# bluenote-1577/skani

Hardware: AMD Instinct MI355X
Metric: genome-pairs/sec (triangle, ~5 Mbp genomes) (higher is better)
Workload: dtype u64

## Files before the change

skani_amd/csrc/chain_dp.h:

```cpp
#pragma once

template <class Co> struct Blk { Co q, r; uint32_t cr; int32_t score; uint32_t root, depth; };

template <int PB, class W>
__global__ __launch_bounds__(256) void chain_dp_kernel(uint32_t n_slots, const Chunk* chunks, uint32_t band, const typename W::Co* anc_q, const typename W::Co* anc_r, unsigned long long* best,
                                                       uint32_t* st ) {
    using Co = typename W::Co; using Blk = skh::Blk<Co>;
    const uint32_t slot = blockIdx.x * (blockDim.x >> 6) + (threadIdx.x >> 6);
    if (slot >= n_slots) return;
    const Chunk ck = chunks[slot];
    if (ck.a_end <= ck.a_begin) return;
    const int l = (int)lane_id();
    Blk prev[PB > 0 ? PB : 1];
#pragma unroll
    for (int b = 0; b < (PB > 0 ? PB : 1); b++) prev[b] = Blk{0, 0, 0, 0, 0, 0};
    for (uint32_t base = ck.a_begin; base < ck.a_end; base += 64) {
        const uint32_t t = base + (uint32_t)l;
        const bool valid = t < ck.a_end;
        Blk cur;
        Co av_q = 0, av_r = 0;
        if (valid) { av_q = anc_q[t]; av_r = anc_r[t]; }
        cur.q = av_q; cur.r = av_r >> 1; cur.cr = (uint32_t)(av_r & 1u);
        cur.score = 0; cur.root = t; cur.depth = 1;
        uint32_t ptr = t;
        uint32_t jlo = base - ck.a_begin > band ? base - band : ck.a_begin;
        const uint32_t jhi = ck.a_end < base + 64 ? ck.a_end : base + 64;
        {
            const Co q_base = anc_q[base];
            uint32_t lo = jlo, hi = base;
            while (lo < hi) { const uint32_t mid = (lo + hi) >> 1; if (anc_q[mid] + BP_CHAIN_BAND < q_base) lo = mid + 1; else hi = mid; }
            jlo = lo;
        }
        for (uint32_t j = jlo; j < jhi; j++) {
            Co qj, rj; uint32_t crj; int32_t sj;
            if (j >= base) {
                const int ln = (int)(j - base);
                const uint32_t pj = wave_readlane(ptr, ln);
                uint32_t rootj = j, depthj = 1;
                if (pj != j) {
                    if (pj >= base) { rootj = wave_readlane(cur.root, (int)(pj - base)); depthj = wave_readlane(cur.depth, (int)(pj - base)) + 1; }
                    else if (PB == 0) { rootj = __atomic_load_n(&st[3 * (size_t)pj + 1], __ATOMIC_RELAXED); depthj = __atomic_load_n(&st[3 * (size_t)pj + 2], __ATOMIC_RELAXED) + 1; }
                    else {
#pragma unroll
                        for (int b = 0; b < PB; b++) {
                            const uint32_t bb = base - 64u * (uint32_t)(b + 1);
                            if (base >= 64u * (uint32_t)(b + 1) && pj >= bb && pj < bb + 64) { rootj = wave_readlane(prev[b].root, (int)(pj - bb)); depthj = wave_readlane(prev[b].depth, (int)(pj - bb)) + 1; }
                        }
                    }
                }
                if (l == ln) { cur.root = rootj; cur.depth = depthj; }
                qj = wave_readlane(cur.q, ln); rj = wave_readlane(cur.r, ln); crj = wave_readlane(cur.cr, ln); sj = wave_readlane(cur.score, ln);
            } else if (PB == 0) {
                const Co rr = anc_r[j];
                qj = anc_q[j]; rj = rr >> 1; crj = (uint32_t)(rr & 1u); sj = (int32_t)__atomic_load_n(&st[3 * (size_t)j], __ATOMIC_RELAXED);
            } else {
                qj = rj = 0; crj = 0; sj = 0;
#pragma unroll
                for (int b = 0; b < PB; b++) {
                    const uint32_t bb = base - 64u * (uint32_t)(b + 1);
                    if (base >= 64u * (uint32_t)(b + 1) && j >= bb && j < bb + 64) {
                        const int ln = (int)(j - bb);
                        qj = wave_readlane(prev[b].q, ln); rj = wave_readlane(prev[b].r, ln); crj = wave_readlane(prev[b].cr, ln); sj = wave_readlane(prev[b].score, ln);
                    }
                }
            }
            if (valid && t > j && t - j <= band && cur.cr == crj) {
                const Co dq = cur.q - qj;
                const bool rev = (crj & 1u) != 0;
                const bool fwd_ok = rev ? (rj > cur.r) : (cur.r > rj);
                const Co dr = rev ? rj - cur.r : cur.r - rj;
                if (dq != 0 && dq <= BP_CHAIN_BAND && fwd_ok && dr <= (Co)MAX_LIN) {
                    const int32_t gap = (int32_t)dr > (int32_t)dq ? (int32_t)(dr - dq) : (int32_t)(dq - dr);
                    const int32_t s = ANCHOR_SCORE - gap + sj;
                    if (gap <= MAX_GAP && s > 0 && s >= cur.score) { cur.score = s; ptr = j; }
                }
            }
        }
        if (valid) atomicMax(&best[cur.root], best_payload((uint32_t)cur.score, t - ck.a_begin, cur.depth));
        if (PB == 0) {
            if (valid) { __atomic_store_n(&st[3 * (size_t)t], (uint32_t)cur.score, __ATOMIC_RELAXED); __atomic_store_n(&st[3 * (size_t)t + 1], cur.root, __ATOMIC_RELAXED); __atomic_store_n(&st[3 * (size_t)t + 2], cur.depth, __ATOMIC_RELAXED); }
            wave_sync_mem();
        }
#pragma unroll
        for (int b = PB - 1; b > 0; b--) prev[b] = prev[b - 1];
        prev[0] = cur;
    }
}

template <class W> struct EmitCtxT { const typename W::Co *anc_q, *anc_r; const PairDesc* pairs; const WidePair* wide; const uint32_t *pc0, *pi0; uint32_t* ivl_cnt; Interval* ivls; uint32_t* err; };
using EmitCtx = EmitCtxT<Narrow>;
__device__ __forceinline__ bool dp_keep(unsigned long long b) {
    const uint32_t sc = (uint32_t)(b >> 40), na = (uint32_t)(b & 0xFFFFFu);
    return na >= MIN_ANCHORS && (int32_t)sc >= MIN_SCORE;
}
template <class W>
__device__ __forceinline__ void dp_write(const Chunk& ck, uint32_t slot, uint32_t p, uint32_t root, unsigned long long b, const EmitCtxT<W>& ec, uint32_t k) {
    using Co = typename W::Co;
    const uint32_t sc = (uint32_t)(b >> 40), bi = (uint32_t)((b >> 20) & 0xFFFFFu), na = (uint32_t)(b & 0xFFFFFu);
    if (ec.pi0[p] + k >= ec.pi0[p + 1]) { atomicAdd(ec.err, 1u); return; }
    const Co ar_q = ec.anc_q[ck.a_begin + root], ar_r = ec.anc_r[ck.a_begin + root], ab_q = ec.anc_q[ck.a_begin + bi], ab_r = ec.anc_r[ck.a_begin + bi];
    const PairDesc& pd = ec.pairs[p];
    const typename W::Arr bo = W::b_goff(pd, ec.wide, p);
    const Co ra = ar_r >> 1, rb = ab_r >> 1;
    const uint32_t rctg = ctg_of(bo, pd.b_nctg, ra); const Co roff = bo[rctg];
    Co qoff = ck.qoff;
    if constexpr (W::wide) qoff = W::a_goff(pd, ec.wide, p)[ck.qctg];
    Interval iv;
    iv.score = sc; iv.na = na; iv.q0 = (uint32_t)(ar_q - qoff); iv.q1 = (uint32_t)(ab_q - qoff);
    iv.r0 = (uint32_t)((ra < rb ? ra : rb) - roff); iv.r1 = (uint32_t)((ra < rb ? rb : ra) - roff);
    iv.rctg = rctg; iv.qctg = ck.qctg; iv.chunk = slot - ec.pc0[p]; iv.rev = (uint32_t)(ar_r & 1u);
    ec.ivls[ec.pi0[p] + k] = iv;
}
template <class W>
__device__ __forceinline__ void dp_emit(const Chunk& ck, uint32_t slot, uint32_t p, uint32_t root, unsigned long long b, const EmitCtxT<W>& ec) {
    if (dp_keep(b)) dp_write(ck, slot, p, root, b, ec, atomicAdd(&ec.ivl_cnt[p], 1u));
}

constexpr uint32_t DP_ORDER_KEYS = 1024, DP_ORDER_BLOCK = 8192;
__device__ __forceinline__ uint32_t dp_order_key(const Chunk& c) { const uint32_t len = c.a_end - c.a_begin; return (DP_ORDER_KEYS - 1u) - (len >= DP_ORDER_KEYS - 1u ? DP_ORDER_KEYS - 1u : len); }
__global__ __launch_bounds__(256) void dp_order_hist_kernel(uint32_t n_slots, const Chunk* chunks, uint32_t* hist) {
    __shared__ uint32_t lh[DP_ORDER_KEYS];
    for (uint32_t x = threadIdx.x; x < DP_ORDER_KEYS; x += 256) lh[x] = 0;
    __syncthreads();
    const uint32_t e = (blockIdx.x + 1u) * DP_ORDER_BLOCK < n_slots ? (blockIdx.x + 1u) * DP_ORDER_BLOCK : n_slots;
    for (uint32_t i = blockIdx.x * DP_ORDER_BLOCK + threadIdx.x; i < e; i += 256) atomicAdd(&lh[dp_order_key(chunks[i])], 1u);
    __syncthreads();
    for (uint32_t x = threadIdx.x; x < DP_ORDER_KEYS; x += 256) if (lh[x]) atomicAdd(&hist[x], lh[x]);
}
__global__ __launch_bounds__(256) void dp_order_scatter_kernel(uint32_t n_slots, const Chunk* chunks, const uint32_t* hist, uint32_t* cursor, uint32_t* order) {
    __shared__ uint32_t base[DP_ORDER_KEYS], mine[DP_ORDER_KEYS]; __shared__ uint32_t wsum[4];
    const uint32_t t = threadIdx.x;
    uint32_t h[4], s = 0;
#pragma unroll
    for (int x = 0; x < 4; x++) { h[x] = hist[4 * t + x]; s += h[x]; mine[4 * t + x] = 0; }
    const uint32_t incl = wave_incl_scan(s);
    if ((t & 63u) == 63u) wsum[t >> 6] = incl;
    __syncthreads();
    uint32_t off = incl - s;
    for (uint32_t w = 0; w < (t >> 6); w++) off += wsum[w];
#pragma unroll
    for (int x = 0; x < 4; x++) { base[4 * t + x] = off; off += h[x]; }
    __syncthreads();
    constexpr int PER = DP_ORDER_BLOCK / 256;
    const uint32_t i0 = blockIdx.x * DP_ORDER_BLOCK + t;
    uint16_t k[PER], r[PER];
#pragma unroll
    for (int x = 0; x < PER; x++) { const uint32_t i = i0 + 256u * x; k[x] = 0xFFFF; if (i < n_slots) { k[x] = (uint16_t)dp_order_key(chunks[i]); r[x] = (uint16_t)atomicAdd(&mine[k[x]], 1u); } }
    __syncthreads();
#pragma unroll
    for (int x = 0; x < 4; x++) { const uint32_t c = 4 * t + x, n = mine[c]; if (n) base[c] += atomicAdd(&cursor[c], n); }
    __syncthreads();
#pragma unroll
    for (int x = 0; x < PER; x++) if (k[x] != 0xFFFF) order[base[k[x]] + r[x]] = i0 + 256u * x;
}

#ifndef DP_EMIT_Q
#define DP_EMIT_Q 6
#endif
#ifndef DP_LINE
#define DP_LINE 8
#endif
template <int NB, int T, uint32_t DP_LDS_SLOTS, bool EXACT, class W = Narrow>
__global__ __launch_bounds__(T) void chain_dp_thread_kernel(uint32_t n_slots, const Chunk* chunks, const uint32_t* chunk_pair, const uint32_t* order, uint32_t band,
                                                            EmitCtxT<W> ec, unsigned long long* spill_best, uint32_t* spill_rr, uint4* emit_q, uint32_t emit_cap) {
    using Co = typename W::Co;
    __shared__ unsigned long long lds_best[DP_LDS_SLOTS * T];
    __shared__ uint32_t lds_rr[DP_LDS_SLOTS * T];
    const uint32_t C = band + 1, tid = threadIdx.x;
    const uint32_t thr = blockIdx.x * T + tid;
    const uint32_t slot = thr < n_slots ? order[thr] : n_slots;
    const size_t n_thr = (size_t)gridDim.x * T;
    auto get_best = [&](uint32_t c) { return c < DP_LDS_SLOTS ? lds_best[c * T + tid] : spill_best[(size_t)(c - DP_LDS_SLOTS) * n_thr + thr]; };
    auto set_best = [&](uint32_t c, unsigned long long v) { if (c < DP_LDS_SLOTS) lds_best[c * T + tid] = v; else spill_best[(size_t)(c - DP_LDS_SLOTS) * n_thr + thr] = v; };
    auto get_rr = [&](uint32_t c) { return c < DP_LDS_SLOTS ? lds_rr[c * T + tid] : spill_rr[(size_t)(c - DP_LDS_SLOTS) * n_thr + thr]; };
    auto set_rr = [&](uint32_t c, uint32_t v) { if (c < DP_LDS_SLOTS) lds_rr[c * T + tid] = v; else spill_rr[(size_t)(c - DP_LDS_SLOTS) * n_thr + thr] = v; };
    Chunk ck{0, 0, 0, 0, 0, 0};
    if (slot < n_slots) ck = chunks[slot];
    const uint32_t n = ck.a_end - ck.a_begin;
    if (n >= MAX_CHUNK_ANCHORS) { atomicAdd(ec.err, 1u); return; }
    const uint32_t p = n ? chunk_pair[slot] : 0;
    uint32_t nq = 0;
    auto emit = [&](uint32_t root, unsigned long long b) {
        if (!dp_keep(b)) return;
        if (NB <= 40 && nq < emit_cap) { emit_q[(size_t)nq * n_thr + thr] = make_uint4(root, (uint32_t)b, (uint32_t)(b >> 32), 0u); nq++; }
        else dp_emit(ck, slot, p, root, b, ec);
    };
    unsigned long long free_mask = C >= 64 ? ~0ull : ((1ull << C) - 1ull);
    uint32_t rq[NB], rr[NB], rs[NB], rd[NB];
    uint32_t rh[W::wide ? NB : 1];
#pragma unroll
    for (int k = 0; k < NB; k++) { rq[k] = 0; rr[k] = 0; rs[k] = 0; rd[k] = 0; }
#pragma unroll
    for (int k = 0; k < (W::wide ? NB : 1); k++) rh[k] = 0;
    constexpr uint32_t LINE = DP_LINE;
    constexpr int APL = W::wide ? 2 : 4;
    constexpr int LQ = LINE / APL;
    __shared__ uint32_t lds_q[LINE * T], lds_r[LINE * T];
    __shared__ uint32_t lds_rh[W::wide ? LINE * T : 1];
    const uint32_t voff = ck.a_begin & (LINE - 1);
    const uint32_t vtot = n ? n + voff : 0;
    const Co* line_q = ec.anc_q + (ck.a_begin - voff); const Co* line_r = ec.anc_r + (ck.a_begin - voff);
    uint4 pq[LQ], pr[LQ];
#pragma unroll
    for (int j = 0; j < LQ; j++) { pq[j] = make_uint4(0, 0, 0, 0); pr[j] = make_uint4(0, 0, 0, 0); }
    if (vtot) {
#pragma unroll
        for (int j = 0; j < LQ; j++) { pq[j] = *(const uint4*)(line_q + APL * j); pr[j] = *(const uint4*)(line_r + APL * j); }
    }
    for (uint32_t v = 0;; v++) {
        const uint32_t kk = v & (LINE - 1);
        if (kk == 0) {
            if (__ballot(v < vtot) == 0) break;
#pragma unroll
            for (int j = 0; j < LQ; j++) {
                if constexpr (W::wide) {
                    lds_q[(2 * j + 0) * T + tid] = pq[j].x; lds_q[(2 * j + 1) * T + tid] = pq[j].z;
                    lds_r[(2 * j + 0) * T + tid] = pr[j].x; lds_r[(2 * j + 1) * T + tid] = pr[j].z;
                    lds_rh[(2 * j + 0) * T + tid] = pr[j].y; lds_rh[(2 * j + 1) * T + tid] = pr[j].w;
                } else {
                    lds_q[(4 * j + 0) * T + tid] = pq[j].x; lds_q[(4 * j + 1) * T + tid] = pq[j].y; lds_q[(4 * j + 2) * T + tid] = pq[j].z; lds_q[(4 * j + 3) * T + tid] = pq[j].w;
                    lds_r[(4 * j + 0) * T + tid] = pr[j].x; lds_r[(4 * j + 1) * T + tid] = pr[j].y; lds_r[(4 * j + 2) * T + tid] = pr[j].z; lds_r[(4 * j + 3) * T + tid] = pr[j].w;
                }
            }
            if (v + LINE < vtot) {
#pragma unroll
                for (int j = 0; j < LQ; j++) { pq[j] = *(const uint4*)(line_q + v + LINE + APL * j); pr[j] = *(const uint4*)(line_r + v + LINE + APL * j); }
            }
        }
        if (v < voff || v >= vtot) continue;
        const uint32_t i = v - voff;
        const uint2 a = make_uint2(lds_q[kk * T + tid], lds_r[kk * T + tid]);
        uint32_t q = a.x, r, sh = 0;
        if constexpr (W::wide) {
            const uint32_t ah = lds_rh[kk * T + tid];
            const uint64_t co = (((uint64_t)ah << 32) | a.y) >> 1, sv = (a.y & 1u) ? ~co : co;
            r = (uint32_t)sv; sh = (uint32_t)(sv >> 32);
        } else r = (a.y & 1u) ? ~(a.y >> 1) : (a.y >> 1);
        int32_t bscore = 0; uint32_t bdc = NONE;
        bool stop = false;
#pragma unroll
        for (int g = 0; g < NB; g += 4) {
            if (g > 0 && !stop) stop = __ballot((int32_t)(q - rq[g - 1]) < (int32_t)BP_CHAIN_BAND) == 0;
            if (!stop) {
#pragma unroll
                for (int k = g; k < g + 4 && k < NB; k++) {
                    if (EXACT || (uint32_t)k < band) {
                        const uint32_t dq1 = q - rq[k], dr1 = r - rr[k];
                        const uint32_t gap = abs_diff_u32(dr1, dq1);
                        const int32_t sc = (int32_t)(rs[k] - gap);
                        bool ok = (dq1 < BP_CHAIN_BAND) & (gap <= (uint32_t)MAX_GAP) & (sc > bscore);
                        if constexpr (W::wide) ok = ok & ((sh - rh[k]) == (r < rr[k] ? 1u : 0u));
                        bscore = ok ? sc : bscore; bdc = ok ? rd[k] : bdc;
                    }
                }
            }
        }
        uint32_t comp, depth;
        if (bdc != NONE) {
            comp = bdc & 0xFFu; depth = (bdc >> 8) + 1;
            set_rr(comp, get_rr(comp) + 1);
            const unsigned long long pay = best_payload((uint32_t)bscore, i, depth);
            if (pay > get_best(comp)) set_best(comp, pay);
        } else {
            comp = (uint32_t)__ffsll((long long)free_mask) - 1u; free_mask &= free_mask - 1ull; depth = 1;
            set_rr(comp, (i << 8) | 1u); set_best(comp, best_payload(0, i, 1));
        }
        uint32_t leaving = rd[NB - 1];
        if (!EXACT) {
#pragma unroll
            for (int k = 0; k < NB; k++) leaving = ((uint32_t)k == band - 1) ? rd[k] : leaving;
        }
        if (i >= band) {
            const uint32_t c_old = leaving & 0xFFu;
            const uint32_t v = get_rr(c_old) - 1u;
            set_rr(c_old, v);
            if ((v & 0xFFu) == 0) { emit(v >> 8, get_best(c_old)); free_mask |= 1ull << c_old; }
        }
#pragma unroll
        for (int k = NB - 1; k > 0; k--) { rq[k] = rq[k - 1]; rr[k] = rr[k - 1]; rs[k] = rs[k - 1]; rd[k] = rd[k - 1]; }
        if constexpr (W::wide) {
#pragma unroll
            for (int k = NB - 1; k > 0; k--) rh[k] = rh[k - 1];
            rh[0] = sh + (r == 0xFFFFFFFFu ? 1u : 0u);
        }
        rq[0] = q + 1u; rr[0] = r + 1u; rs[0] = (uint32_t)(bscore + ANCHOR_SCORE); rd[0] = (depth << 8) | comp;
    }
    const uint32_t live = n < band ? n : band;
#pragma unroll
    for (int k = 0; k < NB; k++) {
        if ((uint32_t)k < live) {
            const uint32_t c_old = rd[k] & 0xFFu;
            const uint32_t v = get_rr(c_old) - 1u;
            set_rr(c_old, v);
            if ((v & 0xFFu) == 0) emit(v >> 8, get_best(c_old));
        }
    }
    if (NB <= 40 && nq) {
        const uint32_t k0 = atomicAdd(&ec.ivl_cnt[p], nq);
        for (uint32_t e = 0; e < nq; e++) {
            const uint4 r = emit_q[(size_t)e * n_thr + thr];
            dp_write(ck, slot, p, r.x, ((unsigned long long)r.z << 32) | r.y, ec, k0 + e);
        }
    }
}

template <class W>
__global__ __launch_bounds__(256) void interval_emit_kernel(uint32_t n_slots, const Chunk* chunks, const unsigned long long* best, const uint32_t* chunk_pair, EmitCtxT<W> ec) {
    const uint32_t slot = blockIdx.x * (blockDim.x >> 6) + (threadIdx.x >> 6);
    if (slot >= n_slots) return;
    const Chunk ck = chunks[slot];
    if (ck.a_end <= ck.a_begin) return;
    const uint32_t p = chunk_pair[slot];
    if (ck.a_end - ck.a_begin >= MAX_CHUNK_ANCHORS) { if (lane_id() == 0) atomicAdd(ec.err, 1u); return; }
    for (uint32_t i = ck.a_begin + lane_id(); i < ck.a_end; i += 64) {
        const unsigned long long b = best[i];
        if (b != 0) dp_emit(ck, slot, p, i - ck.a_begin, b, ec);
    }
}
```

Baseline: 41.83 million.

## Unroll DP line with rotating register ring, drop LDS staging, set waves-per-EU

Fully unrolls the per-line anchor loop with a compile-time static_for. Each step reads its anchor directly from the prefetched uint4 registers instead of staging through shared memory. The band of recent anchors becomes a rotating ring indexed by a compile-time phase, which removes the per-anchor shift of NB registers across the q/r/score/depth arrays; a fix-up rotation runs only when LINE is not a multiple of NB, plus a final runtime rotation of rd. It also adds an amdgpu_waves_per_eu hint per NB and width to steer register allocation. The cost is larger code and a risk of register pressure or spilling, and the post-loop rotation logic is subtle to get right.

```diff
diff --git a/skani_amd/csrc/chain_dp.h b/skani_amd/csrc/chain_dp.h
--- a/skani_amd/csrc/chain_dp.h
+++ b/skani_amd/csrc/chain_dp.h
@@ -160,8 +160,18 @@
 #ifndef DP_LINE
 #define DP_LINE 8
 #endif
+template <int U> struct Idx { static constexpr int value = U; };
+template <int N, int U = 0, class F> __device__ __forceinline__ void static_for(F& f) {
+    if constexpr (U < N) { f(Idx<U>{}); static_for<N, U + 1>(f); }
+}
+#ifdef SKANI_EMU
+#define SKH_DP_WAVES(...)
+#else
+#define SKH_DP_WAVES(...) __attribute__((amdgpu_waves_per_eu(__VA_ARGS__)))
+#endif
+template <int NB, uint32_t LS, class W> constexpr int dp_thread_waves() { return W::wide ? (NB <= 28 ? 2 : 1) : NB <= 20 ? (LS > 1 ? 3 : 2) : NB <= 40 ? 2 : 1; }
 template <int NB, int T, uint32_t DP_LDS_SLOTS, bool EXACT, class W = Narrow>
-__global__ __launch_bounds__(T) void chain_dp_thread_kernel(uint32_t n_slots, const Chunk* chunks, const uint32_t* chunk_pair, const uint32_t* order, uint32_t band,
+__global__ __launch_bounds__(T) SKH_DP_WAVES(dp_thread_waves<NB, DP_LDS_SLOTS, W>()) void chain_dp_thread_kernel(uint32_t n_slots, const Chunk* chunks, const uint32_t* chunk_pair, const uint32_t* order, uint32_t band,
                                                             EmitCtxT<W> ec, unsigned long long* spill_best, uint32_t* spill_rr, uint4* emit_q, uint32_t emit_cap) {
     using Co = typename W::Co;
     __shared__ unsigned long long lds_best[DP_LDS_SLOTS * T];
@@ -195,8 +205,7 @@
     constexpr uint32_t LINE = DP_LINE;
     constexpr int APL = W::wide ? 2 : 4;
     constexpr int LQ = LINE / APL;
-    __shared__ uint32_t lds_q[LINE * T], lds_r[LINE * T];
-    __shared__ uint32_t lds_rh[W::wide ? LINE * T : 1];
+    static_assert(LINE % APL == 0 && (LINE & (LINE - 1)) == 0, "DP_LINE: a power of two, whole 16-byte loads");
     const uint32_t voff = ck.a_begin & (LINE - 1);
     const uint32_t vtot = n ? n + voff : 0;
     const Co* line_q = ec.anc_q + (ck.a_begin - voff); const Co* line_r = ec.anc_r + (ck.a_begin - voff);
@@ -207,83 +216,114 @@
 #pragma unroll
         for (int j = 0; j < LQ; j++) { pq[j] = *(const uint4*)(line_q + APL * j); pr[j] = *(const uint4*)(line_r + APL * j); }
     }
-    for (uint32_t v = 0;; v++) {
-        const uint32_t kk = v & (LINE - 1);
-        if (kk == 0) {
-            if (__ballot(v < vtot) == 0) break;
-#pragma unroll
-            for (int j = 0; j < LQ; j++) {
-                if constexpr (W::wide) {
-                    lds_q[(2 * j + 0) * T + tid] = pq[j].x; lds_q[(2 * j + 1) * T + tid] = pq[j].z;
-                    lds_r[(2 * j + 0) * T + tid] = pr[j].x; lds_r[(2 * j + 1) * T + tid] = pr[j].z;
-                    lds_rh[(2 * j + 0) * T + tid] = pr[j].y; lds_rh[(2 * j + 1) * T + tid] = pr[j].w;
-                } else {
-                    lds_q[(4 * j + 0) * T + tid] = pq[j].x; lds_q[(4 * j + 1) * T + tid] = pq[j].y; lds_q[(4 * j + 2) * T + tid] = pq[j].z; lds_q[(4 * j + 3) * T + tid] = pq[j].w;
-                    lds_r[(4 * j + 0) * T + tid] = pr[j].x; lds_r[(4 * j + 1) * T + tid] = pr[j].y; lds_r[(4 * j + 2) * T + tid] = pr[j].z; lds_r[(4 * j + 3) * T + tid] = pr[j].w;
-                }
-            }
-            if (v + LINE < vtot) {
-#pragma unroll
-                for (int j = 0; j < LQ; j++) { pq[j] = *(const uint4*)(line_q + v + LINE + APL * j); pr[j] = *(const uint4*)(line_r + v + LINE + APL * j); }
-            }
-        }
-        if (v < voff || v >= vtot) continue;
-        const uint32_t i = v - voff;
-        const uint2 a = make_uint2(lds_q[kk * T + tid], lds_r[kk * T + tid]);
-        uint32_t q = a.x, r, sh = 0;
-        if constexpr (W::wide) {
-            const uint32_t ah = lds_rh[kk * T + tid];
-            const uint64_t co = (((uint64_t)ah << 32) | a.y) >> 1, sv = (a.y & 1u) ? ~co : co;
-            r = (uint32_t)sv; sh = (uint32_t)(sv >> 32);
-        } else r = (a.y & 1u) ? ~(a.y >> 1) : (a.y >> 1);
-        int32_t bscore = 0; uint32_t bdc = NONE;
-        bool stop = false;
-#pragma unroll
-        for (int g = 0; g < NB; g += 4) {
-            if (g > 0 && !stop) stop = __ballot((int32_t)(q - rq[g - 1]) < (int32_t)BP_CHAIN_BAND) == 0;
-            if (!stop) {
-#pragma unroll
-                for (int k = g; k < g + 4 && k < NB; k++) {
-                    if (EXACT || (uint32_t)k < band) {
-                        const uint32_t dq1 = q - rq[k], dr1 = r - rr[k];
-                        const uint32_t gap = abs_diff_u32(dr1, dq1);
-                        const int32_t sc = (int32_t)(rs[k] - gap);
-                        bool ok = (dq1 < BP_CHAIN_BAND) & (gap <= (uint32_t)MAX_GAP) & (sc > bscore);
-                        if constexpr (W::wide) ok = ok & ((sh - rh[k]) == (r < rr[k] ? 1u : 0u));
-                        bscore = ok ? sc : bscore; bdc = ok ? rd[k] : bdc;
+    auto ph = [](int u, int k) { return (k + NB - u % NB) % NB; };
+    uint32_t v0 = 0;
+    for (;; v0 += LINE) {
+        if (__ballot(v0 < vtot) == 0) break;
+        uint4 cq[LQ], cr[LQ];
+#pragma unroll
+        for (int j = 0; j < LQ; j++) { cq[j] = pq[j]; cr[j] = pr[j]; }
+        if (v0 + LINE < vtot) {
+#pragma unroll
+            for (int j = 0; j < LQ; j++) { pq[j] = *(const uint4*)(line_q + v0 + LINE + APL * j); pr[j] = *(const uint4*)(line_r + v0 + LINE + APL * j); }
+        }
+        auto step = [&](auto U_) {
+            constexpr int u = decltype(U_)::value;
+            const uint32_t v = v0 + (uint32_t)u;
+            if (v < voff || v >= vtot) return;
+            const uint32_t i = v - voff;
+            auto elem = [&](const uint4& x, int e) { return e == 0 ? x.x : e == 1 ? x.y : e == 2 ? x.z : x.w; };
+            uint32_t q, r, sh = 0;
+            if constexpr (W::wide) {
+                const uint32_t ay = elem(cr[u / 2], 2 * (u & 1)), ah = elem(cr[u / 2], 2 * (u & 1) + 1);
+                q = elem(cq[u / 2], 2 * (u & 1));
+                const uint64_t co = (((uint64_t)ah << 32) | ay) >> 1, sv = (ay & 1u) ? ~co : co;
+                r = (uint32_t)sv; sh = (uint32_t)(sv >> 32);
+            } else {
+                const uint32_t ay = elem(cr[u / 4], u & 3);
+                q = elem(cq[u / 4], u & 3); r = (ay & 1u) ? ~(ay >> 1) : (ay >> 1);
+            }
+            int32_t bscore = 0; uint32_t bdc = NONE;
+            bool stop = false;
+#pragma unroll
+            for (int g = 0; g < NB; g += 4) {
+                if (g > 0 && !stop) stop = __ballot((int32_t)(q - rq[ph(u, g - 1)]) < (int32_t)BP_CHAIN_BAND) == 0;
+                if (!stop) {
+#pragma unroll
+                    for (int k = g; k < g + 4 && k < NB; k++) {
+                        if (EXACT || (uint32_t)k < band) {
+                            const int x = ph(u, k);
+                            const uint32_t dq1 = q - rq[x], dr1 = r - rr[x];
+                            const uint32_t gap = abs_diff_u32(dr1, dq1);
+                            const int32_t sc = (int32_t)(rs[x] - gap);
+                            bool ok = (dq1 < BP_CHAIN_BAND) & (gap <= (uint32_t)MAX_GAP) & (sc > bscore);
+                            if constexpr (W::wide) ok = ok & ((sh - rh[x]) == (r < rr[x] ? 1u : 0u));
+                            bscore = ok ? sc : bscore; bdc = ok ? rd[x] : bdc;
+                        }
                     }
                 }
             }
-        }
-        uint32_t comp, depth;
-        if (bdc != NONE) {
-            comp = bdc & 0xFFu; depth = (bdc >> 8) + 1;
-            set_rr(comp, get_rr(comp) + 1);
-            const unsigned long long pay = best_payload((uint32_t)bscore, i, depth);
-            if (pay > get_best(comp)) set_best(comp, pay);
-        } else {
-            comp = (uint32_t)__ffsll((long long)free_mask) - 1u; free_mask &= free_mask - 1ull; depth = 1;
-            set_rr(comp, (i << 8) | 1u); set_best(comp, best_payload(0, i, 1));
-        }
-        uint32_t leaving = rd[NB - 1];
-        if (!EXACT) {
-#pragma unroll
-            for (int k = 0; k < NB; k++) leaving = ((uint32_t)k == band - 1) ? rd[k] : leaving;
-        }
-        if (i >= band) {
-            const uint32_t c_old = leaving & 0xFFu;
-            const uint32_t v = get_rr(c_old) - 1u;
-            set_rr(c_old, v);
-            if ((v & 0xFFu) == 0) { emit(v >> 8, get_best(c_old)); free_mask |= 1ull << c_old; }
-        }
-#pragma unroll
-        for (int k = NB - 1; k > 0; k--) { rq[k] = rq[k - 1]; rr[k] = rr[k - 1]; rs[k] = rs[k - 1]; rd[k] = rd[k - 1]; }
-        if constexpr (W::wide) {
-#pragma unroll
-            for (int k = NB - 1; k > 0; k--) rh[k] = rh[k - 1];
-            rh[0] = sh + (r == 0xFFFFFFFFu ? 1u : 0u);
-        }
-        rq[0] = q + 1u; rr[0] = r + 1u; rs[0] = (uint32_t)(bscore + ANCHOR_SCORE); rd[0] = (depth << 8) | comp;
+            uint32_t comp, depth;
+            if (bdc != NONE) {
+                comp = bdc & 0xFFu; depth = (bdc >> 8) + 1;
+                set_rr(comp, get_rr(comp) + 1);
+                const unsigned long long pay = best_payload((uint32_t)bscore, i, depth);
+                if (pay > get_best(comp)) set_best(comp, pay);
+            } else {
+                comp = (uint32_t)__ffsll((long long)free_mask) - 1u; free_mask &= free_mask - 1ull; depth = 1;
+                set_rr(comp, (i << 8) | 1u); set_best(comp, best_payload(0, i, 1));
+            }
+            uint32_t leaving = rd[ph(u, NB - 1)];
+            if (!EXACT) {
+#pragma unroll
+                for (int k = 0; k < NB; k++) leaving = ((uint32_t)k == band - 1) ? rd[ph(u, k)] : leaving;
+            }
+            if (i >= band) {
+                const uint32_t c_old = leaving & 0xFFu;
+                const uint32_t v = get_rr(c_old) - 1u;
+                set_rr(c_old, v);
+                if ((v & 0xFFu) == 0) { emit(v >> 8, get_best(c_old)); free_mask |= 1ull << c_old; }
+            }
+            const int o = ph(u, NB - 1);
+            rq[o] = q + 1u; rr[o] = r + 1u; rs[o] = (uint32_t)(bscore + ANCHOR_SCORE); rd[o] = (depth << 8) | comp;
+            if constexpr (W::wide) rh[o] = sh + (r == 0xFFFFFFFFu ? 1u : 0u);
+        };
+        static_for<(int)LINE>(step);
+        constexpr int RS = (int)(LINE % NB);
+        if constexpr (RS != 0) {
+            uint32_t t[NB];
+#pragma unroll
+            for (int k = 0; k < NB; k++) t[k] = rq[(k + NB - RS) % NB];
+#pragma unroll
+            for (int k = 0; k < NB; k++) rq[k] = t[k];
+#pragma unroll
+            for (int k = 0; k < NB; k++) t[k] = rr[(k + NB - RS) % NB];
+#pragma unroll
+            for (int k = 0; k < NB; k++) rr[k] = t[k];
+#pragma unroll
+            for (int k = 0; k < NB; k++) t[k] = rs[(k + NB - RS) % NB];
+#pragma unroll
+            for (int k = 0; k < NB; k++) rs[k] = t[k];
+#pragma unroll
+            for (int k = 0; k < NB; k++) t[k] = rd[(k + NB - RS) % NB];
+#pragma unroll
+            for (int k = 0; k < NB; k++) rd[k] = t[k];
+            if constexpr (W::wide) {
+#pragma unroll
+                for (int k = 0; k < NB; k++) t[k] = rh[(k + NB - RS) % NB];
+#pragma unroll
+                for (int k = 0; k < NB; k++) rh[k] = t[k];
+            }
+        }
+    }
+    const uint32_t post = vtot ? (v0 - vtot) % NB : 0;
+#pragma unroll
+    for (int b = 1; b < NB; b <<= 1) {
+        uint32_t t[NB];
+#pragma unroll
+        for (int k = 0; k < NB; k++) t[k] = (post & (uint32_t)b) ? rd[(k + b) % NB] : rd[k];
+#pragma unroll
+        for (int k = 0; k < NB; k++) rd[k] = t[k];
     }
     const uint32_t live = n < band ? n : band;
 #pragma unroll
```

After: 42.03 million, median of 6. No clear change (+0.5%).
